# mapbox/robosat

Hardware: AMD Instinct MI355X
Metric: 512x512 tiles/sec train+predict, 1/2/4/8 MI355X; mIoU vs CPU ref (higher is better)
Workload: dtype f32; 1 GPU; rs predict ResNet50-UNet, bs=16 3x512x512 fp32 per GPU, 2 classes (BASELINE configs[1]); parallelism=tiles sharded over 1 rank(s), no collective

## Files before the change

robosat_amd/csrc/conv_igemm_dma.hip:

```cpp
#include "conv_igemm_dma_kernel.h"

namespace {

__global__ void pack_dgrad_weight_bf16_kernel(const float* __restrict__ w, bf16_t* __restrict__ out, int Cout, int taps,
                                              int Cin) {
  __shared__ float tile[32][33];
  const int tap = blockIdx.z;
  const int ci0 = blockIdx.x * 32, co0 = blockIdx.y * 32;
  const int tx = threadIdx.x & 31, ty = threadIdx.x >> 5;
  for (int r = ty; r < 32; r += 8) {
    const int co = co0 + r, ci = ci0 + tx;
    tile[r][tx] = (co < Cout && ci < Cin) ? w[((long)co * taps + tap) * Cin + ci] : 0.f;
  }
  __syncthreads();
  const int ftap = taps - 1 - tap;
  for (int r = ty; r < 32; r += 8) {
    const int ci = ci0 + r, co = co0 + tx;
    if (ci < Cin && co < Cout) out[((long)ci * taps + ftap) * Cout + co] = (bf16_t)tile[tx][r];
  }
}

template <typename T>
__global__ __launch_bounds__(256) void weight_prep_kernel(const rs_wprep_item* __restrict__ items, int n) {
  __shared__ float tile[32][33];
// ... 194 lines not shown
  return -1;
}

int halo_mode(const rs_conv_desc* d, bool phase4, int csplit, int epi, int* bn_out, int* bm_out = nullptr) {
  const Tuning tu = tuning();
  if (!tu.halo || (tu.tile != -1 && tu.tile != THALO)) return HALO_NONE;
  bool big = tu.tile == THALO ? tu.rowb == 64 : tu.halo512 != 0;
  const bool c64 = (d->C1 % 64) == 0 && (d->C2 % 64) == 0;
  if ((d->C1 % 32) != 0 || (d->C2 % 32) != 0) return HALO_NONE;
  int bn;
  if (d->Cout % 128 == 0) bn = 128;
  else if (d->Cout > 128 && (long)rs_cdiv(d->Cout, 128) * 128 * 4 <= (long)d->Cout * 5) bn = 128;
  else if (d->Cout % 64 == 0) bn = 64;
  else return HALO_NONE;
  if (csplit > 0 && (csplit % bn) != 0) return HALO_NONE;
  int mode, gh, gw;
  if (phase4) {
    mode = HALO_PHASE, gh = d->Hs, gw = d->Ws;
  } else if (d->ups == 0 && d->kh == 3 && d->kw == 3 && d->stride == 1 && d->pad == 1 && d->Ho == d->Hs && d->Wo == d->Ws) {
    mode = HALO_33, gh = d->Ho, gw = d->Wo;
  } else if (d->ups == 0 && d->kh == 4 && d->kw == 4 && d->stride == 2 && d->pad == 1 && d->Hs == 2 * d->Ho && d->Ws == 2 * d->Wo && d->C2 == 0) {
    mode = HALO_DG4, gh = d->Ho, gw = d->Wo;
  } else {
    return HALO_NONE;
  }
  if (mode != HALO_33 && epi != EPI_EVAL) return HALO_NONE;
  if (tu.tile != THALO && tu.halo512 < 0) big = (long)d->N * (gh / 16) * (gw / 32) >= 256;
  if (big && (bn != 128 || (gh % 16) != 0)) big = false;
  if (!big && !c64) return HALO_NONE;
  const int ph = big ? 16 : 8;
  if ((gh % ph) != 0 || (gw % 32) != 0) return HALO_NONE;
  const long cmax = d->C1 > d->C2 ? d->C1 : d->C2;
  if ((long)d->Hs * d->Ws * cmax * 2 >= (1L << 31)) return HALO_NONE;
  const long blocks = (long)d->N * (gh / ph) * (gw / 32) * rs_cdiv(d->Cout, bn) * (phase4 ? 4 : 1);
  if (tu.tile != THALO) {
    if (blocks < tu.halo_min) return HALO_NONE;
    if (mode == HALO_33 && bn != 128) return HALO_NONE;
    if (mode == HALO_PHASE && d->Cout % 256 == 0) return HALO_NONE;
    if (mode == HALO_DG4 && d->C1 < 128) return HALO_NONE;
  }
  if (bn_out) *bn_out = bn;
  if (bm_out) *bm_out = ph * 32;
  return mode;
}

bool ew_f32_mode(const rs_conv_desc* d, bool phase4, bool plain) {
  const int ew = rs_knobs().conv1x1_ew;
  return ew != 0 && tuning().tile < 0 && !phase4 && plain && rs_conv1x1_ew_f32_ok(d) && (ew > 0 || d->C1 <= 64);
}

bool np_f32_mode(const rs_conv_desc* d, bool phase4, bool plain, bool has_res) {
  const int np = rs_knobs().conv1x1_np;
  return np != 0 && tuning().tile < 0 && !phase4 && plain && rs_conv1x1_np_f32_ok(d) && (np > 0 || (has_res && d->C1 >= 128 && d->C1 <= 512));
}

template <typename T>
int conv_fwd(const rs_conv_desc* d, const void* src1, const void* src2, const void* weight, const float* scale,
             const float* shift, const void* residual, const void* relu_mask, void* out, rs_stream_t stream,
             float* stats = nullptr, const void* bn_y = nullptr, const float* bn_mean = nullptr,
             const float* bn_invstd = nullptr, bool phase4 = false, void* out2 = nullptr, const void* mask2 = nullptr,
             int csplit = 0, const unsigned char* mask_bits = nullptr, float* ws = nullptr, int splits = 0) {
  if (!valid(d) || !src1 || !weight || !out) return RS_EINVAL;
  if (ws && (sizeof(T) != 4 || stats || relu_mask || out2 || mask_bits || splits < 1 || splits != pick_splitk(d, phase4, true))) return RS_EINVAL;
  if (mask_bits && (relu_mask || !bn_y || (d->Cout & 7))) return RS_EINVAL;
  if (out2 && (csplit <= 0 || csplit >= d->Cout || residual || stats)) return RS_EINVAL;
  if (phase4 && (!phase_ok(d) || stats)) return RS_EINVAL;
  if (d->C2 > 0 && !src2) return RS_EINVAL;
  constexpr long ES = (long)sizeof(T);
  if constexpr (sizeof(T) == 2) {
    const int tm = thin_mode(d, phase4, !scale && !shift && !residual && !stats && !out2);
    if (tm >= 0) {
      const int rc = rs_conv_thin_bf16_launch(tm, src1, weight, relu_mask, out, d->N, d->Hs, d->Ws, d->relu, stream);
      if (rc != RS_EINVAL) return rc;
    }
  }
  ConvArgsT<T> a;
  a.src1 = reinterpret_cast<const T*>(src1);
  a.src2 = reinterpret_cast<const T*>(src2);
  a.wgt = reinterpret_cast<const T*>(weight);
  a.scale = scale;
  a.shift = shift;
  a.res = reinterpret_cast<const T*>(residual);
  a.mask = reinterpret_cast<const T*>(relu_mask);
  a.out = reinterpret_cast<T*>(out);
  a.stats = stats;
  a.bn_y = reinterpret_cast<const T*>(bn_y);
  a.bn_mean = bn_mean;
  a.bn_invstd = bn_invstd;
  a.mask_bits = mask_bits;
  a.out2 = reinterpret_cast<T*>(out2);
  a.mask2 = reinterpret_cast<const T*>(mask2);
  a.csplit = csplit;
  a.N = d->N;
  a.Hs = d->Hs;
  a.Ws = d->Ws;
  a.C1 = d->C1;
  a.C2 = d->C2;
  a.phase4 = phase4 ? 1 : 0;
  a.ups = phase4 ? 0 : d->ups;
  a.Hv = a.ups == 0 ? d->Hs : (a.ups == 1 ? 2 * d->Hs : 2 * d->Hs - 1);
  a.Wv = a.ups == 0 ? d->Ws : (a.ups == 1 ? 2 * d->Ws : 2 * d->Ws - 1);
  a.kh = phase4 ? 2 : d->kh;
  a.kw = phase4 ? 2 : d->kw;
  a.stride = d->stride;
  a.pad = d->pad;
  a.Ho = d->Ho;
// ... 35 lines not shown
    if (ws) {
      a.ntiles = rs_cdiv(d->Cout, 64);
      const long rows = M * (phase4 ? 4 : 1);
      const long grid = (long)rs_cdiv(M, 64) * a.ntiles * (phase4 ? 4 : 1) * splits;
      if (grid >= (1L << 31) || rows * d->Cout / 4 >= (1L << 31) * 256) return RS_EINVAL;
      hipStream_t s = (hipStream_t)stream;
      launch(kc == kc128 ? 128 : 64, phase4, EPI_SPLITK, T64x64, (int)grid, s, a);
      splitk_reduce_f32<<<(unsigned)rs_cdiv(rows * (d->Cout / 4), 256), 256, 0, s>>>(ws, splits, rows, (int)M, d->Cout, scale, shift, a.res, a.out, d->relu,
                                                                                phase4 ? 1 : 0, d->Hs * d->Ws, d->Ws, d->Ho, d->Wo);
      return RS_LAUNCH_RESULT();
    }
    if (ew_f32_mode(d, phase4, epi == EPI_EVAL && !relu_mask && !out2 && !mask_bits)) return rs_conv1x1_ew_f32_launch(a, (hipStream_t)stream);
#ifdef RS_EXP_BUILD
    if (np_f32_mode(d, phase4, epi == EPI_EVAL && !relu_mask && !out2 && !mask_bits, residual != nullptr)) return rs_conv1x1_np_f32_launch(a, (hipStream_t)stream);
#endif
  }
  if constexpr (sizeof(T) == 2) {
    int bn = 0, bm = 256;
    const int hm = halo_mode(d, phase4, out2 ? csplit : 0, epi, &bn, &bm);
    if (hm != HALO_NONE) {
      const int gh = hm == HALO_PHASE ? d->Hs : d->Ho, gw = hm == HALO_PHASE ? d->Ws : d->Wo;
      const int ctot = d->C1 + d->C2;
      a.cpt = ctot / (bm == 512 ? 32 : 64);
      a.nk = a.cpt * (hm == HALO_DG4 ? 4 : 1);
      a.Kw = (hm == HALO_PHASE ? 4 : (hm == HALO_33 ? 9 : 16)) * ctot;
      a.tpx = gw / 32;
      a.tpi = a.tpx * (gh / (bm / 32));
      a.ntiles = rs_cdiv(d->Cout, bn);
      const int grid = d->N * a.tpi * a.ntiles * (phase4 ? 4 : 1);
      hipStream_t hs = (hipStream_t)stream;
      if (bm == 512) bn |= 0x1000;
      if (hm == HALO_33) rs_conv_launch_bf16_halo33(bn, epi, grid, hs, a);
#ifdef RS_HALO_KO_BUILD
      else if (hm == HALO_PHASE && bn == 128 && rs_knobs().halo_ko) rs_conv_launch_bf16_halo_phase_ko(rs_knobs().halo_ko, grid, hs, a);
#endif
      else if (hm == HALO_PHASE) rs_conv_launch_bf16_halo_phase(bn, 0, grid, hs, a);
      else rs_conv_launch_bf16_halo_dg4(bn, 0, grid, hs, a);
      return RS_LAUNCH_RESULT();
    }
  }

  const int tile = pick_tile(d, phase4, (int)ES, stats != nullptr);
#ifdef RS_EXP_BUILD
  if constexpr (sizeof(T) == 2) {
    if (rs_knobs().conv1x1_ew_bf16 > 0 && tuning().tile < 0 && epi == EPI_STATS && !phase4 && kTileBM[tile] == 128 &&
        rs_conv1x1_ew_bf16_stats_ok(d))
      return rs_conv1x1_ew_bf16_stats_launch(a, (hipStream_t)stream);
  }
#endif
  if (out2 && (csplit % kTileBN[tile]) != 0) return RS_EINVAL;
  a.ntiles = rs_cdiv(d->Cout, kTileBN[tile]);
  const int grid = rs_cdiv(M, kTileBM[tile]) * a.ntiles * (phase4 ? 4 : 1);
  hipStream_t s = (hipStream_t)stream;
  launch(kc == kc128 ? 128 : 64, phase4, epi, tile, grid, s, a);
  return RS_LAUNCH_RESULT();
}

}

int rs_conv_dma_f32(const rs_conv_desc* d, const float* src1, const float* src2, const float* weight, const float* scale,
                    const float* shift, const float* residual, const float* relu_mask, float* out, void* stream) {
  return conv_fwd<float>(d, src1, src2, weight, scale, shift, residual, relu_mask, out, stream);
}

int rs_conv_dma_tile(const rs_conv_desc* d) { return valid(d) ? pick_tile(d) : RS_EINVAL; }

extern "C" int rs_conv2d_set_tuning(int tile, int rowb) {
  if (tile < -1 || tile >= NTILES || tile == TSTEM_RESERVED || tile == TEW || (rowb != 0 && rowb != 64 && rowb != 128)) return RS_EINVAL;
  rs_knobs().conv_tile = tile;
  rs_knobs().conv_rowb = rowb;
  return 0;
}

extern "C" int rs_conv2d_config(const rs_conv_desc* d, int es, int form, int* tile, int* rowb) {
  if (form < 0 || form > 3) return RS_EINVAL;
  const int phase4 = form & 1;
  const bool plain = (form & 2) == 0;
  if (!valid(d) || (es != 2 && es != 4) || (phase4 && !phase_ok(d))) return RS_EINVAL;
  const int kc128 = 128 / es;
  const bool can128 = d->C1 % kc128 == 0 && d->C2 % kc128 == 0;
  if (es == 2 && thin_mode(d, phase4 != 0, true) >= 0) {
    if (tile) *tile = TTHIN;
    if (rowb) *rowb = d->C1 * 2;
    return 0;
  }
  if (es == 2) {
    int bn = 0, bm = 256;
    if (halo_mode(d, phase4 != 0, 0, EPI_EVAL, &bn, &bm) != HALO_NONE) {
      if (tile) *tile = THALO;
      if (rowb) *rowb = bn | (bm == 512 ? 0x1000 : 0);
      return 0;
    }
  }
  if (es == 4 && ew_f32_mode(d, phase4 != 0, plain)) {
    if (tile) *tile = TEW;
    if (rowb) *rowb = 64;
    return 0;
  }
  if (tile) *tile = pick_tile(d, phase4 != 0, es);
  if (rowb) *rowb = (can128 && pick_rowb(d, es, phase4 != 0) == 128) ? 128 : 64;
  return 0;
}

extern "C" int rs_conv2d_splitk(const rs_conv_desc* d, int form, int* rowb) {
  if (form < 0 || form > 3) return RS_EINVAL;
  const bool phase4 = (form & 1) != 0;
// ... 224 lines not shown
```

robosat_amd/csrc/conv_igemm_dma_kernel.h:

```cpp
#pragma once
#include <stdlib.h>

#include <type_traits>
#include <utility>

#include "lds_dma.h"

enum { EPI_EVAL = 0, EPI_STATS = 1, EPI_BWD = 2, EPI_SPLITK = 3 };
constexpr int kMaxK = 4;
enum Tile { T128x128 = 0, T128x64, T128x32, T64x64, TSTEM_RESERVED, T256x128, T256x256, TTHIN, THALO, TEW, NTILES };
enum { HALO_NONE = 0, HALO_33 = 1, HALO_PHASE = 2, HALO_DG4 = 3 };

template <typename T>
struct ConvArgsT {
  const T* src1;
  const T* src2;
  const T* wgt;
  const float* scale;
  const float* shift;
  const T* res;
  const T* mask;
  T* out;
  union {
    float* stats;
    float* ws;
  };
  const T* bn_y;
  const float* bn_mean;
  const float* bn_invstd;
  const unsigned char* mask_bits;
  T* out2;
  const T* mask2;
  union {
    int csplit;
    int ksplit;
  };
  int N, Hs, Ws, C1, C2, Hv, Wv, ups;
  int kh, kw, stride, pad, Ho, Wo, Cout;
  int M, cpt, nk, Kw, relu, ntiles, ntaps, phase4;
  int tpx, tpi;
};


#define RS_CONV_LAUNCHER(name, T) \
  __attribute__((visibility("hidden"))) void name(int tile, int rowb, int grid, hipStream_t s, const ConvArgsT<T>& a)
RS_CONV_LAUNCHER(rs_conv_launch_f32_plain_eval, float);
RS_CONV_LAUNCHER(rs_conv_launch_f32_plain_stats, float);
RS_CONV_LAUNCHER(rs_conv_launch_f32_plain_bwd, float);
RS_CONV_LAUNCHER(rs_conv_launch_f32_phase_eval, float);
RS_CONV_LAUNCHER(rs_conv_launch_f32_plain_splitk, float);
RS_CONV_LAUNCHER(rs_conv_launch_f32_phase_splitk, float);
RS_CONV_LAUNCHER(rs_conv_launch_bf16_plain_eval, bf16_t);
RS_CONV_LAUNCHER(rs_conv_launch_bf16_plain_stats, bf16_t);
RS_CONV_LAUNCHER(rs_conv_launch_bf16_plain_bwd, bf16_t);
RS_CONV_LAUNCHER(rs_conv_launch_bf16_phase_eval, bf16_t);
RS_CONV_LAUNCHER(rs_conv_launch_bf16_halo33, bf16_t);
RS_CONV_LAUNCHER(rs_conv_launch_bf16_halo_phase, bf16_t);
RS_CONV_LAUNCHER(rs_conv_launch_bf16_halo_dg4, bf16_t);
__attribute__((visibility("hidden"))) void rs_conv_launch_bf16_halo_phase_ko(int ko, int grid, hipStream_t s, const ConvArgsT<bf16_t>& a);
__attribute__((visibility("hidden"))) int rs_conv1x1_ew_f32_ok(const rs_conv_desc* d);
__attribute__((visibility("hidden"))) int rs_conv1x1_ew_f32_launch(const ConvArgsT<float>& a, hipStream_t s);
__attribute__((visibility("hidden"))) int rs_conv1x1_np_f32_ok(const rs_conv_desc* d);
__attribute__((visibility("hidden"))) int rs_conv1x1_np_f32_launch(const ConvArgsT<float>& a, hipStream_t s);
__attribute__((visibility("hidden"))) int rs_conv1x1_ew_bf16_stats_ok(const rs_conv_desc* d);
__attribute__((visibility("hidden"))) int rs_conv1x1_ew_bf16_stats_launch(const ConvArgsT<bf16_t>& a, hipStream_t s);

#ifdef RS_CONV_INSTANTIATE
namespace {

template <typename T>
struct Piece;
template <>
struct Piece<float> {
  __device__ static __forceinline__ void load(const float* p, float (&v)[4]) {
    const f32x4 t = *reinterpret_cast<const f32x4*>(p);
#pragma unroll
    for (int e = 0; e < 4; ++e) v[e] = t[e];
  }
  __device__ static __forceinline__ void round(const float (&v)[4], float (&w)[4]) {
#pragma unroll
    for (int e = 0; e < 4; ++e) w[e] = v[e];
  }
  __device__ static __forceinline__ void store(float* p, const float (&v)[4]) {
    f32x4 t;
#pragma unroll
    for (int e = 0; e < 4; ++e) t[e] = v[e];
    *reinterpret_cast<f32x4*>(p) = t;
  }
};
template <>
struct Piece<bf16_t> {
  __device__ static __forceinline__ void load(const bf16_t* p, float (&v)[8]) {
    const bf16x8 t = *reinterpret_cast<const bf16x8*>(p);
#pragma unroll
    for (int e = 0; e < 8; ++e) v[e] = (float)t[e];
  }
  __device__ static __forceinline__ void round(const float (&v)[8], float (&w)[8]) {
#pragma unroll
    for (int e = 0; e < 8; ++e) w[e] = (float)(bf16_t)v[e];
  }
  __device__ static __forceinline__ void store(bf16_t* p, const float (&v)[8]) {
    bf16x8 t;
#pragma unroll
    for (int e = 0; e < 8; ++e) t[e] = (bf16_t)v[e];
    *reinterpret_cast<bf16x8*>(p) = t;
  }
};

__device__ __forceinline__ void mma16(f32x16& acc, const u32x4 a, const u32x4 b, bf16_t) {
  acc = __builtin_amdgcn_mfma_f32_32x32x16_bf16(__builtin_bit_cast(bf16x8, a), __builtin_bit_cast(bf16x8, b), acc, 0, 0, 0);
}
__device__ __forceinline__ void mma16(f32x16& acc, const u32x4 a, const u32x4 b, float) {
  const f32x4 fa = __builtin_bit_cast(f32x4, a), fb = __builtin_bit_cast(f32x4, b);
#pragma unroll
  for (int t = 0; t < 4; ++t) acc = __builtin_amdgcn_mfma_f32_32x32x2f32(fa[t], fb[t], acc, 0, 0, 0);
}

constexpr unsigned int kDmaClamp = 0xFFFE0000u;
constexpr int kDmaOOB = (int)0xFFFF0000u;
static_assert((unsigned int)kDmaOOB > kDmaClamp && (unsigned int)kDmaOOB - kDmaClamp == 0x10000u && 0u - (unsigned int)kDmaOOB == 0x10000u,
              "the sentinel is out of range for every descriptor, with 64 KiB for soff on either side");

template <class F, int... I>
__device__ __forceinline__ void rb_for_each(F&& f, std::integer_sequence<int, I...>) {
  (f(std::integral_constant<int, I>()), ...);
}
constexpr int halo_tap_of_piece(int j, int ntap, int njh) { return j * (ntap - 2) / njh; }
constexpr int halo_pieces_at_tap(int t, int ntap, int njh) {
  int n = 0;
  for (int j = 0; j < njh; ++j) n += halo_tap_of_piece(j, ntap, njh) == t ? 1 : 0;
  return n;
}

constexpr int conv_waves_per_simd(int nw, int bm, int bn, int rowb, int es, int epi, int halo = 0) {
  if (halo) return 2;
  const int lds = 2 * (bm + bn) * rowb + 9 * bm * 4;
  const int blocks = 160 * 1024 / lds;
  const int w = blocks * nw / 4;
  const int cap = nw == 8 ? (bm * bn >= 256 * 256 ? 1 : 2) : ((es == 4 && epi == 2 && bm * bn >= 128 * 128) ? 2 : 4);
  return w < 1 ? 1 : (w > cap ? cap : w);
}

template <typename T, int BM, int BN, int WGM, int WGN, int ROWB, bool PHASE, int EPI, int HALO = HALO_NONE, int KO = 0>
__global__ __launch_bounds__(64 * WGM * WGN, conv_waves_per_simd(WGM * WGN, BM, BN, ROWB, (int)sizeof(T), EPI, HALO)) void conv_igemm_dma(
    const ConvArgsT<T> p) {
  static_assert(WGM * WGN == 4 || WGM * WGN == 8, "4 or 8 waves per block");
  static_assert(ROWB == 128 || ROWB == 64, "a K-chunk is a 128- or 64-byte row");
  constexpr int NBUF = 2;
  constexpr int NW = WGM * WGN;
  constexpr int NT = 64 * NW;
  constexpr int ES = (int)sizeof(T);
  constexpr int EPP = 16 / ES;
  constexpr int KC = ROWB / ES;
  constexpr int WM = BM / WGM, WN = BN / WGN;
  constexpr int TM = WM / 32, TN = WN / 32;
  constexpr int CPR = ROWB / 16;
  constexpr int RI = 64 / CPR;
  constexpr int IA = BM / RI, IB = BN / RI;
  constexpr int NI = (IA + IB + NW - 1) / NW;
  constexpr int KS = CPR / 2;
  constexpr int BUF = (BM + BN) * ROWB;
  constexpr int LDO = BN + 4;
  constexpr bool HL = HALO != HALO_NONE;
  constexpr int PWD = 32, PHT = BM / 32;
  constexpr int HK = HALO == HALO_33 ? 3 : 2;
  constexpr int HNT = HK * HK;
  constexpr int HWD = PWD + HK - 1, HHT = PHT + HK - 1, HROWS = HHT * HWD;
  constexpr int NJH = ((HROWS + RI - 1) / RI + NW - 1) / NW;
  constexpr int HALOB = ((HROWS + RI - 1) / RI) * 1024;
  constexpr int HSCRATCH = 2 * HALOB;
  constexpr int HBOFF = 2 * HALOB + 1024;
  constexpr int DRING = 4;
  constexpr int BSLOT = BN * ROWB;
  constexpr int NBW = IB / NW;
  constexpr int PIPE = HL ? HBOFF + DRING * BSLOT : NBUF * BUF;
  constexpr int STAGE = WGM * 32 * LDO * 4;
  constexpr int MAINB = PIPE > STAGE ? PIPE : STAGE;
  constexpr int TABN = HL ? BM : (2 * kMaxK + 1) * BM;
  static_assert(TM >= 1 && TN >= 1, "wave tile must hold one 32x32 MFMA tile");
  static_assert((IA % NW) == 0 && IB >= 1 && (BM % RI) == 0 && (BN % RI) == 0, "DMA instruction split");
  static_assert(!HL || (sizeof(T) == 2 && NW == 8 && (IB % NW) == 0 && WM % 32 == 0 && HNT >= 4 && KS % 2 == 0 && (HALO == HALO_PHASE) == PHASE),
                "halo forms: bf16, 8 waves, whole weight DMA instructions per wave");
  static_assert(MAINB + TABN * 4 <= 160 * 1024, "LDS");
  constexpr bool SPLIT = EPI == EPI_SPLITK;
  constexpr bool STATS = EPI == EPI_STATS || EPI == EPI_BWD;
  static_assert(!SPLIT || (ES == 4 && !HL), "split K: the fp32 implicit-GEMM forms");

  __shared__ __attribute__((aligned(16))) unsigned char smem[MAINB + TABN * 4];
  int* taby = reinterpret_cast<int*>(smem + MAINB);
  int* tabx = taby + kMaxK * BM;
  int* orow = HL ? taby : tabx + kMaxK * BM;

  const int tid = threadIdx.x;
  const int lane = tid & 63;
  const int wave = __builtin_amdgcn_readfirstlane(tid >> 6);
  const int wm = wave / WGN, wn = wave % WGN;

  int bid = rs_xcd_remap(blockIdx.x, gridDim.x);
  int py = 0, px = 0;
  if (PHASE) {
    py = (bid >> 1) & 1;
    px = bid & 1;
    bid >>= 2;
  }
  int ksl = 0;
  if constexpr (SPLIT) {
    const int tps = (int)(gridDim.x >> (PHASE ? 2 : 0)) / p.ksplit;
    ksl = bid / tps;
    bid -= ksl * tps;
  }
  const int mt = bid / p.ntiles, nt = bid - mt * p.ntiles;
  const int m0 = mt * BM, n0 = nt * BN;

  const int Hd = PHASE ? p.Hs : p.Ho, Wd = PHASE ? p.Ws : p.Wo;
  const int HdWd = Hd * Wd;
  int hn = 0, hy0 = 0, hx0 = 0;
  if constexpr (HL) {
    hn = __builtin_amdgcn_readfirstlane(mt / p.tpi);
    const int rem = mt - hn * p.tpi;
    const int ty = __builtin_amdgcn_readfirstlane(rem / p.tpx);
    hy0 = ty * PHT;
    hx0 = (rem - ty * p.tpx) * PWD;
  }
  const int nfirst = HL ? hn : __builtin_amdgcn_readfirstlane(m0 / HdWd);
  const int ush = p.ups ? 1 : 0;
  const int upar = p.ups == 2 ? 1 : 0;
  const int pad_y = PHASE ? 1 - py : p.pad, pad_x = PHASE ? 1 - px : p.pad;

  if constexpr (HL) {
    for (int e = tid; e < BM; e += NT) {
      const int y = hy0 + e / PWD, x = hx0 + e % PWD;
      int v = -1;
      if (y < Hd && x < Wd) v = PHASE ? (hn * p.Ho + 2 * y + py) * p.Wo + 2 * x + px : (hn * Hd + y) * Wd + x;
      orow[e] = v;
    }
  }
  for (int e = tid; e < (HL ? 0 : (p.kh + p.kw + 1) * BM); e += NT) {
    const int t = e / BM, row = e - t * BM;
    const int m = m0 + row;
    int v = -1;
    if (m < p.M) {
      const int n = m / HdWd;
      const int rem = m - n * HdWd;
      const int oy = rem / Wd;
      const int ox = rem - oy * Wd;
      if (t < p.kh) {
        const int iy = oy * p.stride - pad_y + t;
        if (((unsigned)iy < (unsigned)p.Hv) && ((iy & upar) == 0)) v = ((n - nfirst) * p.Hs + (iy >> ush)) * p.Ws;
      } else if (t < p.kh + p.kw) {
        const int ix = ox * p.stride - pad_x + (t - p.kh);
        if (((unsigned)ix < (unsigned)p.Wv) && ((ix & upar) == 0)) v = ix >> ush;
      } else {
        v = PHASE ? (n * p.Ho + 2 * oy + py) * p.Wo + 2 * ox + px : m;
      }
    }
    if (t < p.kh) taby[t * BM + row] = v;
    else if (t < p.kh + p.kw) tabx[(t - p.kh) * BM + row] = v;
    else orow[row] = v;
  }

  const long img1 = (long)p.Hs * p.Ws * p.C1;
  const long img2 = (long)p.Hs * p.Ws * p.C2;
  const __amdgpu_buffer_rsrc_t rsrc1 = rs_dma_rsrc<kDmaClamp>(p.src1 + nfirst * img1, (long)(p.N - nfirst) * img1 * ES);
  const __amdgpu_buffer_rsrc_t rsrc2 = rs_dma_rsrc<kDmaClamp>(p.C2 ? p.src2 + nfirst * img2 : p.src1, (long)(p.N - nfirst) * img2 * ES);
  const __amdgpu_buffer_rsrc_t rsrcw =
      rs_dma_rsrc<kDmaClamp>(p.wgt + (long)(2 * py + px) * p.Cout * p.Kw, (long)p.Cout * p.Kw * ES);

  const int ra = lane / CPR, pp = lane % CPR;
  const int fsw = ROWB == 128 ? ((4 * (wave & 1) + (ra >> 1)) & 7) : ((ra >> 2) & 3);
  const int gp = pp ^ fsw;
  const unsigned int lds0 = __builtin_amdgcn_readfirstlane(rs_lds_addr(smem));
  constexpr int NIA = IA / NW;
  int wrow[NI];
#pragma unroll
  for (int j = 0; j < NI; ++j) wrow[j] = ((n0 + RI * (wave + NW * j - IA) + ra) * p.Kw + gp * EPP) * ES;
  __syncthreads();

  int pbase[NIA];
  auto load_tap = [&](int (&dst)[NIA], int r, int s_, bool first) __attribute__((always_inline)) {
    const int cs2 = (first ? p.C1 : p.C2) * ES;
#pragma unroll
    for (int j = 0; j < NIA; ++j) {
      const int row = RI * (wave + NW * j) + ra;
      const int y = taby[r * BM + row], x = tabx[s_ * BM + row];
      dst[j] = (y | x) < 0 ? kDmaOOB : (y + x) * cs2 + gp * 16;
    }
  };
  int lr = 0, ls = 0, lc = 0, lk = 0;
  int nkl = p.nk;
  if constexpr (SPLIT) {
    const int u32 = KC == 32 ? 1 : 2, n32 = p.nk / u32;
    const int k0 = (int)((long)ksl * n32 / p.ksplit) * u32, k1 = (int)((long)(ksl + 1) * n32 / p.ksplit) * u32;
    nkl = k1 - k0;
    lk = k0;
    const int tap = k0 / p.cpt;
    lc = k0 - tap * p.cpt;
    lr = tap / p.kw;
    ls = tap - lr * p.kw;
    if (lc != 0) load_tap(pbase, lr, ls, lc * KC < p.C1);
  }
  unsigned int fL = lds0;
  __amdgpu_buffer_rsrc_t frs = rsrc1;
  int fsa = 0, fsb = 0;
  auto begin_chunk = [&](int buf) __attribute__((always_inline)) {
    const int c0 = lc * KC;
    const bool first = c0 < p.C1;
    if (lc == 0 || c0 == p.C1) load_tap(pbase, lr, ls, first);
    fL = lds0 + buf * BUF;
    frs = first ? rsrc1 : rsrc2;
    fsa = (first ? c0 : c0 - p.C1) * ES;
    fsb = lk * ROWB;
    ++lk;
    ++lc;
    const int w1 = (lc == p.cpt) ? 1 : 0;
    lc = w1 ? 0 : lc;
    ls += w1;
    const int w2 = (ls == p.kw) ? 1 : 0;
    ls = w2 ? 0 : ls;
    lr += w2;
  };
  auto issue_piece = [&](int j) __attribute__((always_inline)) {
    const int ii = wave + NW * j;
    if (j < NIA) {
      rs_dma16(frs, fL + ii * 1024, pbase[j], fsa);
    } else if ((IB % NW) == 0 || ii < IA + IB) {
      rs_dma16(rsrcw, fL + ii * 1024, wrow[j], fsb);
    }
  };

  f32x16 acc[TN][TM];
#pragma unroll
  for (int a = 0; a < TN; ++a)
#pragma unroll
    for (int b = 0; b < TM; ++b)
#pragma unroll
      for (int r = 0; r < 16; ++r) acc[a][b][r] = 0.f;

  const int frow = lane & 31;
  const int fl = ROWB == 128 ? ((frow >> 1) & 7) : ((frow >> 2) & 3);
  int foff[KS];
#pragma unroll
  for (int s = 0; s < KS; ++s) foff[s] = ((2 * s + (lane >> 5)) ^ fl) * 16;
  const int abase = (wm * WM + frow) * ROWB;
  const int bbase = (BM + wn * WN + frow) * ROWB;

  auto read_frag = [&](const unsigned char* L, int s, u32x4 (&a)[TM], u32x4 (&b)[TN]) __attribute__((always_inline)) {
#pragma unroll
    for (int tm = 0; tm < TM; ++tm) a[tm] = *reinterpret_cast<const u32x4*>(L + abase + 32 * tm * ROWB + foff[s]);
#pragma unroll
    for (int tn = 0; tn < TN; ++tn) b[tn] = *reinterpret_cast<const u32x4*>(L + bbase + 32 * tn * ROWB + foff[s]);
  };
  if constexpr (!HL) {
  if (nkl > 0) {
    begin_chunk(0);
#pragma unroll
    for (int q = 0; q < NI; ++q) issue_piece(q);
  }
  }
  constexpr int NMMA = KS * TM * TN;
  constexpr int PSTEP = NMMA / (2 * NI) >= 1 ? NMMA / (2 * NI) : 1;
  constexpr int PIN = (NMMA + PSTEP - 1) / PSTEP < NI ? (NMMA + PSTEP - 1) / PSTEP : NI;
  auto chunk = [&](int kc, auto fetch_tag) __attribute__((always_inline)) {
    constexpr bool FETCH = decltype(fetch_tag)::value;
    rs_dma_wait();
    __syncthreads();
    if (FETCH) begin_chunk((kc + 1) % NBUF);
    const unsigned char* L = smem + (kc % NBUF) * BUF;
    u32x4 fa[2][TM], fb[2][TN];
    read_frag(L, 0, fa[0], fb[0]);
#pragma unroll
    for (int s = 0; s < KS; ++s) {
      if (s + 1 < KS) read_frag(L, s + 1, fa[(s + 1) & 1], fb[(s + 1) & 1]);
#pragma unroll
      for (int tm = 0; tm < TM; ++tm)
#pragma unroll
        for (int tn = 0; tn < TN; ++tn) {
          const int q = (s * TM + tm) * TN + tn;
          if (FETCH && q % PSTEP == 0 && q / PSTEP < PIN) issue_piece(q / PSTEP);
          mma16(acc[tn][tm], fb[s & 1][tn], fa[s & 1][tm], T());
        }
    }
    if (FETCH) {
#pragma unroll
      for (int q = PIN; q < NI; ++q) issue_piece(q);
    }
  };
  if constexpr (!HL) {
    int kc = 0;
    for (; kc < nkl - 1; ++kc) chunk(kc, std::true_type());
    for (; kc < nkl; ++kc) chunk(kc, std::false_type());
  } else {
    constexpr int RPT = WM / 32;
    constexpr int NHI = (HROWS + RI - 1) / RI;
    const int hi = lane >> 5, l31 = lane & 31;
    const int ctot = p.C1 + p.C2;
    int ho1[NJH], ho2[NJH];
    auto halo_pix = [&](int pa, int pb) __attribute__((always_inline)) {
      int hpix[NJH];
#pragma unroll
      for (int j = 0; j < NJH; ++j) {
        const int R = RI * (wave + NW * j) + ra;
        const int hyy = R / HWD, hxx = R - hyy * HWD;
        int v = -1;
        if (HALO == HALO_DG4) {
          const int su = hy0 - pa + hyy, sv = hx0 - pb + hxx;
          if (R < HROWS && (unsigned)su < (unsigned)p.Ho && (unsigned)sv < (unsigned)p.Wo) v = (2 * su + pa) * p.Ws + 2 * sv + pb;
        } else {
          const int sy = hy0 - pad_y + hyy, sx = hx0 - pad_x + hxx;
          if (R < HROWS && (unsigned)sy < (unsigned)p.Hs && (unsigned)sx < (unsigned)p.Ws) v = sy * p.Ws + sx;
        }
// ... 129 lines not shown
              }
            };
            constexpr int toff = (t / HK) * HWD + (t % HK);
            constexpr int tn1 = (t + 1) % HNT;
            constexpr int toff1 = (tn1 / HK) * HWD + (tn1 % HK);
            const int hbuf1 = (t + 1 < HNT) ? hbuf : nbuf;
            const int slot = gstep & (DRING - 1), slot1 = (gstep + 1) & (DRING - 1);
#pragma unroll
            for (int ks = 0; ks < KS; ++ks) {
              if constexpr (KO != 3) {
                if (ks + 1 < KS) rd(hbuf, slot, toff, ks + 1, fa[(ks + 1) & 1], fb[(ks + 1) & 1], t);
                else rd(hbuf1, slot1, toff1, 0, fa[0], fb[0], tn1);
              }
#pragma unroll
              for (int tm = 0; tm < TM; ++tm)
#pragma unroll
                for (int tn = 0; tn < TN; ++tn) {
                  const int i = (ks * TM + tm) * TN + tn;
                  if (i % PST == 0 && i / PST < NP) piece(i / PST);
                  if constexpr (KO == 4) {
                    asm volatile("" ::"v"(fb[ks & 1][tn]), "v"(fa[ks & 1][tm]));
                  } else if constexpr (KO == 3) {
                    mma16(acc[tn][tm], fb[0][tn], fa[0][tm], T());
                  } else {
                    mma16(acc[tn][tm], fb[ks & 1][tn], fa[ks & 1][tm], T());
                  }
                }
            }
#pragma unroll
            for (int i = (NMMA + PST - 1) / PST; i < NP; ++i) piece(i);
          },
          std::make_integer_sequence<int, HNT>());
      cur = nxt;
      nxt = group(q + 2);
      if (HALO == HALO_DG4) halo_pix(nxt.pa, nxt.pb);
    }
    rs_dma_wait();
    __builtin_amdgcn_sched_barrier(0);
  }
  __syncthreads();
  if constexpr (HL) __builtin_amdgcn_sched_barrier(0);

  float* lds = reinterpret_cast<float*>(smem);
  constexpr int TPR = BN / EPP;
  constexpr int RPI = NT / TPR;
  const int cc = tid % TPR, rr = tid / TPR;
  const int col = n0 + cc * EPP;
  const bool cvalid = col < p.Cout;
  constexpr int NSC = EPI == EPI_EVAL ? EPP : 1, NST = EPI == EPI_EVAL ? 1 : EPP, NBN = EPI == EPI_BWD ? EPP : 1;
  float sc[NSC], sh[NSC];
  if constexpr (EPI == EPI_EVAL) {
#pragma unroll
    for (int e = 0; e < EPP; ++e) {
      sc[e] = (p.scale && cvalid) ? p.scale[col + e] : 1.f;
      sh[e] = (p.shift && cvalid) ? p.shift[col + e] : 0.f;
    }
  }
  T* outp = p.out;
  if constexpr (SPLIT) outp = p.ws;
  const T* maskp = p.mask;
  int ostride = p.Cout, ocol = col;
  if (EPI == EPI_EVAL && p.out2) {
    if (n0 >= p.csplit) {
      outp = p.out2;
      maskp = p.mask2;
      ostride = p.Cout - p.csplit;
      ocol = col - p.csplit;
    } else {
      ostride = p.csplit;
    }
  }
  float st0[NST], st1[NST];
  float bmu[NBN], bis[NBN];
#pragma unroll
  for (int e = 0; e < NST; ++e) st0[e] = st1[e] = 0.f;
  if constexpr (EPI == EPI_BWD) {
#pragma unroll
    for (int e = 0; e < EPP; ++e) {
      bmu[e] = cvalid ? p.bn_mean[col + e] : 0.f;
      bis[e] = cvalid ? p.bn_invstd[col + e] : 0.f;
    }
  }
  constexpr int NIT = WN / (2 * EPP);
  constexpr int G = (ES == 4 && EPI == EPI_BWD) ? 1 : 2;
  static_assert(NIT * RPI == WGM * 32 && NIT % G == 0, "row groups tile the pass");
  const bool has_res = EPI != EPI_STATS && !SPLIT && p.res != nullptr, has_mask = EPI != EPI_STATS && !SPLIT && maskp != nullptr;
  const bool has_bits = EPI == EPI_BWD && p.mask_bits != nullptr;
  constexpr bool has_bny = EPI == EPI_BWD;
  auto load_group = [&](int tm, int g0, long (&o)[G], bool (&ok)[G], u32x4 (&rr_)[G], u32x4 (&rm_)[G], u32x4 (&ry_)[G])
      __attribute__((always_inline)) {
#pragma unroll
    for (int i = 0; i < G; ++i) {
      const int lrow = rr + (g0 + i) * RPI;
      const int row = (lrow >> 5) * WM + 32 * tm + (lrow & 31);
      const int opix = orow[row];
      ok[i] = opix >= 0 && cvalid;
      if constexpr (SPLIT) o[i] = ok[i] ? (((long)ksl * (PHASE ? 4 : 1) + (2 * py + px)) * p.M + m0 + row) * p.Cout + col : 0;
      else o[i] = ok[i] ? (long)opix * ostride + ocol : 0;
    }
    if (has_res) {
#pragma unroll
      for (int i = 0; i < G; ++i) rr_[i] = *reinterpret_cast<const u32x4*>(p.res + o[i]);
    }
    if (has_mask) {
#pragma unroll
      for (int i = 0; i < G; ++i) rm_[i] = *reinterpret_cast<const u32x4*>(maskp + o[i]);
    }
    if constexpr (EPI == EPI_BWD) {
      if (has_bits) {
#pragma unroll
        for (int i = 0; i < G; ++i) rm_[i][0] = p.mask_bits[o[i] >> 3];
      }
    }
    if constexpr (has_bny) {
#pragma unroll
      for (int i = 0; i < G; ++i) ry_[i] = *reinterpret_cast<const u32x4*>(p.bn_y + o[i]);
    }
  };
  auto unpack = [&](const u32x4 raw, float (&v)[EPP]) __attribute__((always_inline)) {
    if constexpr (ES == 4) {
      const f32x4 t = __builtin_bit_cast(f32x4, raw);
#pragma unroll
      for (int e = 0; e < 4; ++e) v[e] = t[e];
    } else {
      const bf16x8 t = __builtin_bit_cast(bf16x8, raw);
#pragma unroll
      for (int e = 0; e < 8; ++e) v[e] = (float)t[e];
    }
  };
  auto finish_group = [&](int g0, const long (&o)[G], const bool (&ok)[G], const u32x4 (&rr_)[G], const u32x4 (&rm_)[G],
                          const u32x4 (&ry_)[G]) __attribute__((always_inline)) {
#pragma unroll
    for (int i = 0; i < G; ++i) {
      const int lrow = rr + (g0 + i) * RPI;
      float v[EPP];
#pragma unroll
      for (int h = 0; h < EPP / 4; ++h) {
        const f32x4 t = *reinterpret_cast<const f32x4*>(&lds[lrow * LDO + cc * EPP + 4 * h]);
#pragma unroll
        for (int e = 0; e < 4; ++e) v[4 * h + e] = EPI == EPI_EVAL ? t[e] * sc[(4 * h + e) % NSC] + sh[(4 * h + e) % NSC] : t[e];
      }
      if (has_res) {
        float r[EPP];
        unpack(rr_[i], r);
#pragma unroll
        for (int e = 0; e < EPP; ++e) v[e] += r[e];
      }
      if (EPI == EPI_EVAL && p.relu) {
#pragma unroll
        for (int e = 0; e < EPP; ++e) v[e] = fmaxf(v[e], 0.f);
      }
      if (has_mask) {
        float z[EPP];
        unpack(rm_[i], z);
#pragma unroll
        for (int e = 0; e < EPP; ++e) v[e] = z[e] > 0.f ? v[e] : 0.f;
      }
      if constexpr (EPI == EPI_BWD) {
        if (has_bits) {
          const unsigned int bits = EPP == 8 ? rm_[i][0] : (rm_[i][0] >> (o[i] & 4));
#pragma unroll
          for (int e = 0; e < EPP; ++e) v[e] = ((bits >> e) & 1u) ? v[e] : 0.f;
        }
      }
      if (ok[i]) Piece<T>::store(outp + o[i], v);
      if constexpr (STATS) {
        float w[EPP];
        Piece<T>::round(v, w);
        const float keep = ok[i] ? 1.f : 0.f;
        if constexpr (EPI == EPI_BWD) {
          float yv[EPP];
          unpack(ry_[i], yv);
#pragma unroll
          for (int e = 0; e < EPP; ++e) {
            st0[e % NST] += keep * w[e];
            st1[e % NST] += keep * (w[e] * ((yv[e] - bmu[e % NBN]) * bis[e % NBN]));
          }
        } else {
#pragma unroll
          for (int e = 0; e < EPP; ++e) {
            st0[e % NST] += keep * w[e];
            st1[e % NST] += keep * (w[e] * w[e]);
          }
        }
      }
    }
  };
#pragma unroll
  for (int tm = 0; tm < TM; ++tm) {
    long o[G];
    bool ok[G];
    u32x4 rr_[G], rm_[G], ry_[G];
    load_group(tm, 0, o, ok, rr_, rm_, ry_);
    if (tm > 0) __syncthreads();
    {
      const int pr = wm * 32 + (lane & 31);
      const int ccol = wn * WN + 4 * (lane >> 5);
#pragma unroll
      for (int tn = 0; tn < TN; ++tn)
#pragma unroll
        for (int g = 0; g < 4; ++g) {
// ... 2 lines not shown
          v[1] = acc[tn][tm][4 * g + 1];
          v[2] = acc[tn][tm][4 * g + 2];
          v[3] = acc[tn][tm][4 * g + 3];
          *reinterpret_cast<f32x4*>(&lds[pr * LDO + ccol + 32 * tn + 8 * g]) = v;
        }
    }
    __syncthreads();
    finish_group(0, o, ok, rr_, rm_, ry_);
#pragma unroll
    for (int g0 = G; g0 < NIT; g0 += G) {
      load_group(tm, g0, o, ok, rr_, rm_, ry_);
      finish_group(g0, o, ok, rr_, rm_, ry_);
    }
  }
  if constexpr (STATS) {
    __syncthreads();
    float* r0 = lds;
    float* r1 = lds + RPI * BN;
#pragma unroll
    for (int e = 0; e < EPP; ++e) {
      r0[rr * BN + cc * EPP + e] = st0[e % NST];
      r1[rr * BN + cc * EPP + e] = st1[e % NST];
    }
    __syncthreads();
    if (tid < 2 * BN) {
      const float* r = tid < BN ? r0 : r1;
      const int c = tid < BN ? tid : tid - BN;
      float a = 0.f;
#pragma unroll 4
      for (int l = 0; l < RPI; ++l) a += r[l * BN + c];
      if (n0 + c < p.Cout) p.stats[((long)mt * 2 + (tid < BN ? 0 : 1)) * p.Cout + n0 + c] = a;
    }
  }
}


template <typename T, int ROWB, bool PHASE, int EPI>
void launch_rows(int tile, int grid, hipStream_t s, const ConvArgsT<T>& a) {
  if constexpr (sizeof(T) == 2 && EPI == EPI_EVAL) {
    if (tile == T256x256) {
      conv_igemm_dma<T, 256, 256, 2, 4, ROWB, PHASE, EPI><<<grid, 512, 0, s>>>(a);
      return;
    }
  }
  switch (tile) {
    case T128x128: conv_igemm_dma<T, 128, 128, 2, 2, ROWB, PHASE, EPI><<<grid, 256, 0, s>>>(a); break;
    case T128x64: conv_igemm_dma<T, 128, 64, 2, 2, ROWB, PHASE, EPI><<<grid, 256, 0, s>>>(a); break;
    case T128x32: conv_igemm_dma<T, 128, 32, 4, 1, ROWB, PHASE, EPI><<<grid, 256, 0, s>>>(a); break;
    case T256x128: conv_igemm_dma<T, 256, 128, 4, 2, ROWB, PHASE, EPI><<<grid, 512, 0, s>>>(a); break;
    default: conv_igemm_dma<T, 64, 64, 2, 2, ROWB, PHASE, EPI><<<grid, 256, 0, s>>>(a); break;
  }
}

template <int ROWB, bool PHASE>
void launch_splitk(int grid, hipStream_t s, const ConvArgsT<float>& a) {
  conv_igemm_dma<float, 64, 64, 2, 2, ROWB, PHASE, EPI_SPLITK><<<grid, 256, 0, s>>>(a);
}

}

template <int HALO, bool PHASE, int EPI>
void launch_halo(int bn, int grid, hipStream_t s, const ConvArgsT<bf16_t>& a) {
  if (bn == (128 | 0x1000)) conv_igemm_dma<bf16_t, 512, 128, 4, 2, 64, PHASE, EPI, HALO><<<grid, 512, 0, s>>>(a);
  else if (bn == 128) conv_igemm_dma<bf16_t, 256, 128, 4, 2, 128, PHASE, EPI, HALO><<<grid, 512, 0, s>>>(a);
  else conv_igemm_dma<bf16_t, 256, 64, 4, 2, 128, PHASE, EPI, HALO><<<grid, 512, 0, s>>>(a);
}

#define RS_CONV_DEFINE_LAUNCHER(name, T, PHASE, EPI)                                            \
  void name(int tile, int rowb, int grid, hipStream_t s, const ConvArgsT<T>& a) {               \
    if (rowb == 128) launch_rows<T, 128, PHASE, EPI>(tile, grid, s, a);                         \
    else launch_rows<T, 64, PHASE, EPI>(tile, grid, s, a);                                      \
  }
#define RS_CONV_DEFINE_SPLITK_LAUNCHER(name, PHASE)                                              \
  void name(int, int rowb, int grid, hipStream_t s, const ConvArgsT<float>& a) {                \
    if (rowb == 128) launch_splitk<128, PHASE>(grid, s, a);                                     \
    else launch_splitk<64, PHASE>(grid, s, a);                                                  \
  }
#endif
```

Measured before the change: 1708 tiles/s.

## Specialize fp32 eval conv epilogues by kind and add 1x1 direct-addressing path

Adds compile-time epilogue kinds (affine, relu, residual+relu) for fp32 eval convolutions so runtime branches on relu, mask and out2 disappear, and scale/shift are loaded early as vectors. For unit-stride 1x1 convs without padding or upsampling, a FAST1 variant skips building the per-row pixel index tables, drops a barrier and addresses input rows directly. This adds template instantiations and new translation units, which raises compile time and code size, and the residual path changes epilogue grouping, which may affect register pressure.

```diff
diff --git a/robosat_amd/csrc/conv_igemm_dma.hip b/robosat_amd/csrc/conv_igemm_dma.hip
--- a/robosat_amd/csrc/conv_igemm_dma.hip
+++ b/robosat_amd/csrc/conv_igemm_dma.hip
@@ -270,6 +270,13 @@
 bool np_f32_mode(const rs_conv_desc* d, bool phase4, bool plain, bool has_res) {
   const int np = rs_knobs().conv1x1_np;
   return np != 0 && tuning().tile < 0 && !phase4 && plain && rs_conv1x1_np_f32_ok(d) && (np > 0 || (has_res && d->C1 >= 128 && d->C1 <= 512));
+}
+
+int eval_kind(const float* scale, const float* shift, bool res, bool mask_or_out2, int relu, int epi, bool phase4) {
+  if ((RS_EVAL_TILE_STEPS & 2) == 0 || epi != EPI_EVAL || phase4 || !scale || !shift || mask_or_out2) return EK_RT;
+  if ((((unsigned long)scale | (unsigned long)shift) & 15) != 0) return EK_RT;
+  if (res) return relu ? EK_RES_RELU : EK_RT;
+  return relu ? EK_RELU : EK_AFFINE;
 }
 
 template <typename T>
@@ -411,6 +418,15 @@
   a.ntiles = rs_cdiv(d->Cout, kTileBN[tile]);
   const int grid = rs_cdiv(M, kTileBM[tile]) * a.ntiles * (phase4 ? 4 : 1);
   hipStream_t s = (hipStream_t)stream;
+  if constexpr (sizeof(T) == 4) {
+    const int ek = eval_kind(scale, shift, a.res != nullptr, a.mask != nullptr || out2 != nullptr, d->relu, epi, phase4);
+    if (ek != EK_RT) {
+      const bool fast1 = (RS_EVAL_TILE_STEPS & 4) != 0 && d->kh == 1 && d->kw == 1 && d->stride == 1 && d->pad == 0 && d->ups == 0 && d->C2 == 0 &&
+                         d->Ho == d->Hs && d->Wo == d->Ws;
+      auto* const kind_launch = ek == EK_AFFINE ? rs_conv_launch_f32_eval_affine : (ek == EK_RELU ? rs_conv_launch_f32_eval_relu : rs_conv_launch_f32_eval_res_relu);
+      if (kind_launch(fast1 ? 1 : 0, tile, kc == kc128 ? 128 : 64, grid, s, a) == 0) return RS_LAUNCH_RESULT();
+    }
+  }
   launch(kc == kc128 ? 128 : 64, phase4, epi, tile, grid, s, a);
   return RS_LAUNCH_RESULT();
 }
diff --git a/robosat_amd/csrc/conv_igemm_dma_f32_eval_affine.hip b/robosat_amd/csrc/conv_igemm_dma_f32_eval_affine.hip
--- /dev/null
+++ b/robosat_amd/csrc/conv_igemm_dma_f32_eval_affine.hip
@@ -0,0 +1,4 @@
+#define RS_CONV_INSTANTIATE
+#include "conv_igemm_dma_kernel.h"
+
+RS_CONV_DEFINE_KIND_LAUNCHER(rs_conv_launch_f32_eval_affine, EK_AFFINE)
diff --git a/robosat_amd/csrc/conv_igemm_dma_f32_eval_relu.hip b/robosat_amd/csrc/conv_igemm_dma_f32_eval_relu.hip
--- /dev/null
+++ b/robosat_amd/csrc/conv_igemm_dma_f32_eval_relu.hip
@@ -0,0 +1,4 @@
+#define RS_CONV_INSTANTIATE
+#include "conv_igemm_dma_kernel.h"
+
+RS_CONV_DEFINE_KIND_LAUNCHER(rs_conv_launch_f32_eval_relu, EK_RELU)
diff --git a/robosat_amd/csrc/conv_igemm_dma_f32_eval_res_relu.hip b/robosat_amd/csrc/conv_igemm_dma_f32_eval_res_relu.hip
--- /dev/null
+++ b/robosat_amd/csrc/conv_igemm_dma_f32_eval_res_relu.hip
@@ -0,0 +1,4 @@
+#define RS_CONV_INSTANTIATE
+#include "conv_igemm_dma_kernel.h"
+
+RS_CONV_DEFINE_KIND_LAUNCHER(rs_conv_launch_f32_eval_res_relu, EK_RES_RELU)
diff --git a/robosat_amd/csrc/conv_igemm_dma_kernel.h b/robosat_amd/csrc/conv_igemm_dma_kernel.h
--- a/robosat_amd/csrc/conv_igemm_dma_kernel.h
+++ b/robosat_amd/csrc/conv_igemm_dma_kernel.h
@@ -10,6 +10,11 @@
 constexpr int kMaxK = 4;
 enum Tile { T128x128 = 0, T128x64, T128x32, T64x64, TSTEM_RESERVED, T256x128, T256x256, TTHIN, THALO, TEW, NTILES };
 enum { HALO_NONE = 0, HALO_33 = 1, HALO_PHASE = 2, HALO_DG4 = 3 };
+enum { EK_RT = 0, EK_AFFINE = 1, EK_RELU = 2, EK_RES_RELU = 3 };
+constexpr int conv_epix(int epi, int ek, bool fast1) { return epi | (ek << 4) | (fast1 ? 0x100 : 0); }
+#ifndef RS_EVAL_TILE_STEPS
+#define RS_EVAL_TILE_STEPS 7
+#endif
 
 template <typename T>
 struct ConvArgsT {
@@ -45,6 +50,11 @@
 #define RS_CONV_LAUNCHER(name, T) \
   __attribute__((visibility("hidden"))) void name(int tile, int rowb, int grid, hipStream_t s, const ConvArgsT<T>& a)
 RS_CONV_LAUNCHER(rs_conv_launch_f32_plain_eval, float);
+#define RS_CONV_KIND_LAUNCHER(name) \
+  __attribute__((visibility("hidden"))) int name(int fast1, int tile, int rowb, int grid, hipStream_t s, const ConvArgsT<float>& a)
+RS_CONV_KIND_LAUNCHER(rs_conv_launch_f32_eval_affine);
+RS_CONV_KIND_LAUNCHER(rs_conv_launch_f32_eval_relu);
+RS_CONV_KIND_LAUNCHER(rs_conv_launch_f32_eval_res_relu);
 RS_CONV_LAUNCHER(rs_conv_launch_f32_plain_stats, float);
 RS_CONV_LAUNCHER(rs_conv_launch_f32_plain_bwd, float);
 RS_CONV_LAUNCHER(rs_conv_launch_f32_phase_eval, float);
@@ -141,9 +151,14 @@
   return w < 1 ? 1 : (w > cap ? cap : w);
 }
 
-template <typename T, int BM, int BN, int WGM, int WGN, int ROWB, bool PHASE, int EPI, int HALO = HALO_NONE, int KO = 0>
-__global__ __launch_bounds__(64 * WGM * WGN, conv_waves_per_simd(WGM * WGN, BM, BN, ROWB, (int)sizeof(T), EPI, HALO)) void conv_igemm_dma(
+template <typename T, int BM, int BN, int WGM, int WGN, int ROWB, bool PHASE, int EPIX, int HALO = HALO_NONE, int KO = 0>
+__global__ __launch_bounds__(64 * WGM * WGN, conv_waves_per_simd(WGM * WGN, BM, BN, ROWB, (int)sizeof(T), EPIX & 15, HALO)) void conv_igemm_dma(
     const ConvArgsT<T> p) {
+  constexpr int EPI = EPIX & 15;
+  constexpr int EK = (EPIX >> 4) & 15;
+  constexpr bool FAST1 = (EPIX & 0x100) != 0;
+  constexpr bool EARLY = EK != EK_RT && (RS_EVAL_TILE_STEPS & 1) != 0;
+  static_assert(EPIX == EPI || (sizeof(T) == 4 && EPI == EPI_EVAL && HALO == HALO_NONE && !PHASE), "fixed kinds / FAST1: the fp32 direct-form EVAL launches");
   static_assert(WGM * WGN == 4 || WGM * WGN == 8, "4 or 8 waves per block");
   static_assert(ROWB == 128 || ROWB == 64, "a K-chunk is a 128- or 64-byte row");
   constexpr int NBUF = 2;
@@ -222,7 +237,7 @@
     hy0 = ty * PHT;
     hx0 = (rem - ty * p.tpx) * PWD;
   }
-  const int nfirst = HL ? hn : __builtin_amdgcn_readfirstlane(m0 / HdWd);
+  const int nfirst = HL ? hn : (FAST1 ? 0 : __builtin_amdgcn_readfirstlane(m0 / HdWd));
   const int ush = p.ups ? 1 : 0;
   const int upar = p.ups == 2 ? 1 : 0;
   const int pad_y = PHASE ? 1 - py : p.pad, pad_x = PHASE ? 1 - px : p.pad;
@@ -235,7 +250,7 @@
       orow[e] = v;
     }
   }
-  for (int e = tid; e < (HL ? 0 : (p.kh + p.kw + 1) * BM); e += NT) {
+  for (int e = tid; e < ((HL || FAST1) ? 0 : (p.kh + p.kw + 1) * BM); e += NT) {
     const int t = e / BM, row = e - t * BM;
     const int m = m0 + row;
     int v = -1;
@@ -261,8 +276,10 @@
 
   const long img1 = (long)p.Hs * p.Ws * p.C1;
   const long img2 = (long)p.Hs * p.Ws * p.C2;
-  const __amdgpu_buffer_rsrc_t rsrc1 = rs_dma_rsrc<kDmaClamp>(p.src1 + nfirst * img1, (long)(p.N - nfirst) * img1 * ES);
-  const __amdgpu_buffer_rsrc_t rsrc2 = rs_dma_rsrc<kDmaClamp>(p.C2 ? p.src2 + nfirst * img2 : p.src1, (long)(p.N - nfirst) * img2 * ES);
+  const __amdgpu_buffer_rsrc_t rsrc1 = FAST1 ? rs_dma_rsrc<kDmaClamp>(p.src1 + (long)m0 * p.C1, (long)(p.M - m0) * p.C1 * ES)
+                                             : rs_dma_rsrc<kDmaClamp>(p.src1 + nfirst * img1, (long)(p.N - nfirst) * img1 * ES);
+  const __amdgpu_buffer_rsrc_t rsrc2 =
+      FAST1 ? rsrc1 : rs_dma_rsrc<kDmaClamp>(p.C2 ? p.src2 + nfirst * img2 : p.src1, (long)(p.N - nfirst) * img2 * ES);
   const __amdgpu_buffer_rsrc_t rsrcw =
       rs_dma_rsrc<kDmaClamp>(p.wgt + (long)(2 * py + px) * p.Cout * p.Kw, (long)p.Cout * p.Kw * ES);
 
@@ -274,7 +291,7 @@
   int wrow[NI];
 #pragma unroll
   for (int j = 0; j < NI; ++j) wrow[j] = ((n0 + RI * (wave + NW * j - IA) + ra) * p.Kw + gp * EPP) * ES;
-  __syncthreads();
+  if constexpr (!FAST1) __syncthreads();
 
   int pbase[NIA];
   auto load_tap = [&](int (&dst)[NIA], int r, int s_, bool first) __attribute__((always_inline)) {
@@ -286,6 +303,13 @@
       dst[j] = (y | x) < 0 ? kDmaOOB : (y + x) * cs2 + gp * 16;
     }
   };
+  if constexpr (FAST1) {
+#pragma unroll
+    for (int j = 0; j < NIA; ++j) {
+      const int row = RI * (wave + NW * j) + ra;
+      pbase[j] = m0 + row < p.M ? row * (p.C1 * ES) + gp * 16 : kDmaOOB;
+    }
+  }
   int lr = 0, ls = 0, lc = 0, lk = 0;
   int nkl = p.nk;
   if constexpr (SPLIT) {
@@ -303,6 +327,12 @@
   __amdgpu_buffer_rsrc_t frs = rsrc1;
   int fsa = 0, fsb = 0;
   auto begin_chunk = [&](int buf) __attribute__((always_inline)) {
+    if constexpr (FAST1) {
+      fL = lds0 + buf * BUF;
+      fsa = fsb = lk * ROWB;
+      ++lk;
+      return;
+    }
     const int c0 = lc * KC;
     const bool first = c0 < p.C1;
     if (lc == 0 || c0 == p.C1) load_tap(pbase, lr, ls, first);
@@ -356,6 +386,12 @@
 #pragma unroll
     for (int q = 0; q < NI; ++q) issue_piece(q);
   }
+  }
+  f32x4 scv = {1.f, 1.f, 1.f, 1.f}, shv = {0.f, 0.f, 0.f, 0.f};
+  if constexpr (EARLY) {
+    const int ecol = n0 + (tid % (BN / EPP)) * EPP;
+    scv = *reinterpret_cast<const f32x4*>(p.scale + (ecol < p.Cout ? ecol : 0));
+    shv = *reinterpret_cast<const f32x4*>(p.shift + (ecol < p.Cout ? ecol : 0));
   }
   constexpr int NMMA = KS * TM * TN;
   constexpr int PSTEP = NMMA / (2 * NI) >= 1 ? NMMA / (2 * NI) : 1;
@@ -591,15 +627,20 @@
   if constexpr (EPI == EPI_EVAL) {
 #pragma unroll
     for (int e = 0; e < EPP; ++e) {
-      sc[e] = (p.scale && cvalid) ? p.scale[col + e] : 1.f;
-      sh[e] = (p.shift && cvalid) ? p.shift[col + e] : 0.f;
+      if constexpr (EARLY) {
+        sc[e] = scv[e % 4];
+        sh[e] = shv[e % 4];
+      } else {
+        sc[e] = (p.scale && cvalid) ? p.scale[col + e] : 1.f;
+        sh[e] = (p.shift && cvalid) ? p.shift[col + e] : 0.f;
+      }
     }
   }
   T* outp = p.out;
   if constexpr (SPLIT) outp = p.ws;
   const T* maskp = p.mask;
   int ostride = p.Cout, ocol = col;
-  if (EPI == EPI_EVAL && p.out2) {
+  if (EPI == EPI_EVAL && EK == EK_RT && p.out2) {
     if (n0 >= p.csplit) {
       outp = p.out2;
       maskp = p.mask2;
@@ -621,9 +662,12 @@
     }
   }
   constexpr int NIT = WN / (2 * EPP);
-  constexpr int G = (ES == 4 && EPI == EPI_BWD) ? 1 : 2;
+  constexpr int GRES = TM * TN * 16 + NIT * EPP > 80 ? NIT / 2 : NIT;
+  constexpr int G = (ES == 4 && EPI == EPI_BWD) ? 1 : ((EARLY && EK == EK_RES_RELU) ? GRES : 2);
   static_assert(NIT * RPI == WGM * 32 && NIT % G == 0, "row groups tile the pass");
-  const bool has_res = EPI != EPI_STATS && !SPLIT && p.res != nullptr, has_mask = EPI != EPI_STATS && !SPLIT && maskp != nullptr;
+  const bool has_res = EK != EK_RT ? EK == EK_RES_RELU : (EPI != EPI_STATS && !SPLIT && p.res != nullptr);
+  const bool has_mask = EK == EK_RT && EPI != EPI_STATS && !SPLIT && maskp != nullptr;
+  const bool do_relu = EK != EK_RT ? EK != EK_AFFINE : (EPI == EPI_EVAL && p.relu != 0);
   const bool has_bits = EPI == EPI_BWD && p.mask_bits != nullptr;
   constexpr bool has_bny = EPI == EPI_BWD;
   auto load_group = [&](int tm, int g0, long (&o)[G], bool (&ok)[G], u32x4 (&rr_)[G], u32x4 (&rm_)[G], u32x4 (&ry_)[G])
@@ -632,7 +676,7 @@
     for (int i = 0; i < G; ++i) {
       const int lrow = rr + (g0 + i) * RPI;
       const int row = (lrow >> 5) * WM + 32 * tm + (lrow & 31);
-      const int opix = orow[row];
+      const int opix = FAST1 ? (m0 + row < p.M ? m0 + row : -1) : orow[row];
       ok[i] = opix >= 0 && cvalid;
       if constexpr (SPLIT) o[i] = ok[i] ? (((long)ksl * (PHASE ? 4 : 1) + (2 * py + px)) * p.M + m0 + row) * p.Cout + col : 0;
       else o[i] = ok[i] ? (long)opix * ostride + ocol : 0;
@@ -685,7 +729,7 @@
 #pragma unroll
         for (int e = 0; e < EPP; ++e) v[e] += r[e];
       }
-      if (EPI == EPI_EVAL && p.relu) {
+      if (do_relu) {
 #pragma unroll
         for (int e = 0; e < EPP; ++e) v[e] = fmaxf(v[e], 0.f);
       }
@@ -794,6 +838,18 @@
   }
 }
 
+template <int ROWB, int EK, bool FAST1>
+int launch_eval_kind(int tile, int grid, hipStream_t s, const ConvArgsT<float>& a) {
+  constexpr int X = conv_epix(EPI_EVAL, EK, FAST1);
+  switch (tile) {
+    case T128x128: conv_igemm_dma<float, 128, 128, 2, 2, ROWB, false, X><<<grid, 256, 0, s>>>(a); return 0;
+    case T128x64: conv_igemm_dma<float, 128, 64, 2, 2, ROWB, false, X><<<grid, 256, 0, s>>>(a); return 0;
+    case T128x32: conv_igemm_dma<float, 128, 32, 4, 1, ROWB, false, X><<<grid, 256, 0, s>>>(a); return 0;
+    case T64x64: conv_igemm_dma<float, 64, 64, 2, 2, ROWB, false, X><<<grid, 256, 0, s>>>(a); return 0;
+    default: return RS_EINVAL;
+  }
+}
+
 template <int ROWB, bool PHASE>
 void launch_splitk(int grid, hipStream_t s, const ConvArgsT<float>& a) {
   conv_igemm_dma<float, 64, 64, 2, 2, ROWB, PHASE, EPI_SPLITK><<<grid, 256, 0, s>>>(a);
@@ -813,6 +869,11 @@
     if (rowb == 128) launch_rows<T, 128, PHASE, EPI>(tile, grid, s, a);                         \
     else launch_rows<T, 64, PHASE, EPI>(tile, grid, s, a);                                      \
   }
+#define RS_CONV_DEFINE_KIND_LAUNCHER(name, EK)                                                                    \
+  int name(int fast1, int tile, int rowb, int grid, hipStream_t s, const ConvArgsT<float>& a) {                   \
+    if (fast1) return rowb == 128 ? launch_eval_kind<128, EK, true>(tile, grid, s, a) : launch_eval_kind<64, EK, true>(tile, grid, s, a);  \
+    return rowb == 128 ? launch_eval_kind<128, EK, false>(tile, grid, s, a) : launch_eval_kind<64, EK, false>(tile, grid, s, a);           \
+  }
 #define RS_CONV_DEFINE_SPLITK_LAUNCHER(name, PHASE)                                              \
   void name(int, int rowb, int grid, hipStream_t s, const ConvArgsT<float>& a) {                \
     if (rowb == 128) launch_splitk<128, PHASE>(grid, s, a);                                     \
```

Result: faster. 1732 tiles/s, median of 6 (+1.4%).
